# Dunni3/FlowMol

Hardware: AMD Instinct MI355X
Metric: molecules/sec at 250 timesteps (GEOM-drugs-sized graphs) (higher is better)
Workload: dtype f32

## Files before the change

flowmol_amd/csrc/fm_engine.cpp:

```cpp
#include "fm_host.h"

namespace fmh { thread_local std::string g_create_error; }

namespace {

struct Blob {
    const float* base; const fm_tensor_desc* t; int n;
    std::string err;
    const float* get(const std::string& name, int64_t d0, int64_t d1 = -1) {
        for (int i = 0; i < n; ++i)
            if (name == t[i].name) {
                const bool ok = (d1 < 0) ? (t[i].ndim == 1 && t[i].shape[0] == d0)
                                         : (t[i].ndim == 2 && t[i].shape[0] == d0 && t[i].shape[1] == d1);
                if (!ok) {
                    char b[256];
                    snprintf(b, sizeof b, "tensor %s: shape (%lld,%lld) != expected (%lld,%lld)", name.c_str(),
                             (long long)t[i].shape[0], (long long)(t[i].ndim > 1 ? t[i].shape[1] : -1), (long long)d0, (long long)d1);
                    if (err.empty()) err = b;
                    return nullptr;
                }
                return base + t[i].offset;
            }
        if (err.empty()) err = "missing tensor " + name;
        return nullptr;
// ... 184 lines not shown
        else launch_mlp(L, mode_n, node, a, wn, N, p.small_node ? 16 : FM_TM);
        if (pair) launch_mlp(L, mode_p, pair, e, wp, U, p.small_pair ? 16 : pair32 ? 32 : FM_TM);
    }
}

void launch_node_proj(Launch& L, const char* name, int V, bool small, int N, const FmProjArgs& pa) {
    const int tm = small ? 16 : FM_TM;
    launch_inst(L, node_proj_instances, {V, tm}, name, dim3((N + tm - 1) / tm), dim3(FM_THREADS), lds_proj(V, tm), pa);
}

int evaluate(fm_ctx* c, hipStream_t st, const fm_state* state, const fm_dst* prev, int remove_com, const fm_dst* out,
             bool taps_on, const fm_dense_state* dense = nullptr, const float* temb = nullptr) {
    Launch L{c, st};
    const BatchPlan& p = c->plan;
    const int V = c->V, TE = p.tm_edge, TN = p.tm_node, HX = c->HX;
    const FmBatch& b = c->b;
    const int N = b.N, E = b.E, U = b.U;
    const fm_config& cf = c->cfg;
    const int nc1 = c->nc + 1;
    auto tap = [&](const std::string& n, const void* src, size_t bytes) { if (taps_on) L.tap(n, src, bytes); };

    const bool mlp4 = p.mlp4 && !dense;
    const int n_pq = (prev && !dense) ? p.n_pq : 0;
    FmMlpArgs ma{};
    ma.na = c->na; ma.nc = c->nc; ma.ne = c->ne;
    ma.rbf_mu_step = c->rbf_mu_step; ma.rbf_inv_sigma = c->rbf_inv_sigma;
    const float* x_t = dense ? dense->x_t : state->x_t;
    if (dense) {
        const int kp = c->node_embed.K1p;
        L("dense_in", fm_k_dense_node_in, dim3(std::min(2048, (int)(((size_t)N * kp + 255) / 256))), dim3(256), 0, c->Ps, kp, N,
          (const float*)dense->a_t, c->na, (const float*)dense->c_t, c->nc, temb, cf.time_embedding_dim);
        FmMlpArgs a{};
        a.in = c->Ps; a.in_ld = kp; a.out = c->s; a.out_ld = 256; a.ln_g = c->node_ln_g; a.ln_b = c->node_ln_b; a.ln_n = c->S;
        launch_mlp(L, FM_MLP_TABLE, "embed_nodes", a, c->node_embed, N);
        FmMlpArgs e{};
        e.in = dense->e_t; e.in_ld = c->ne; e.in_w = c->ne; e.out = c->ef; e.out_ld = 128; e.ln_g = c->edge_ln_g; e.ln_b = c->edge_ln_b; e.ln_n = c->F;
        e.p_e0 = b.p_e0; e.p_e1 = b.p_e1;
        launch_mlp(L, FM_MLP_TABLE, "embed_pairs", e, c->edge_embed, U);
        tap("embed.s", c->s, (size_t)N * 256 * 4);
        tap("embed.ef", c->ef, (size_t)E * 128 * 4);
    } else if (prev) {
        FmMlpArgs a = ma;
        a.s_tab = c->s_tab; a.tok_a = state->a_t; a.tok_c = state->c_t; a.n_c1 = nc1;
        a.prev_a = prev->a; a.prev_c = prev->c; a.prev_x = prev->x; a.x_t = state->x_t;
        a.out = c->s;
        FmMlpArgs e = ma;
        e.e_src = b.e_src; e.e_dst = b.e_dst; e.e_pair = b.e_pair; e.tok_e = state->e_t;
        e.prev_e = prev->e; e.prev_x = prev->x; e.x_t = state->x_t; e.T1 = c->T1; e.ef_tab = c->ef_tab;
        e.out = c->ef;
        e.p_e0 = b.p_e0; e.p_e1 = b.p_e1;
        if (n_pq > 0) {
            e.slabW0 = c->conv[0].Ws_slab; e.slabQ0 = c->Q[0];
            if (n_pq > 1) { e.slabW1 = c->conv[1].Ws_slab; e.slabQ1 = c->Q[1]; }
        }
        FmMlp4Args a4{};
        a4.N = N; a4.W1q = c->sc_node_W1q; a4.b1 = c->sc_node.b1; a4.W2q = c->sc_node_W2q; a4.b2 = c->sc_node.b2;
        a4.s_tab = a.s_tab; a4.tok_a = a.tok_a; a4.tok_c = a.tok_c; a4.n_c1 = nc1; a4.prev_a = a.prev_a; a4.prev_c = a.prev_c; a4.prev_x = a.prev_x; a4.x_t = a.x_t;
        a4.na = c->na; a4.nc = c->nc; a4.rbf_mu_step = c->rbf_mu_step; a4.rbf_inv_sigma = c->rbf_inv_sigma; a4.out = c->s;
        launch_mlp_stage(L, p, mlp4, FM_MLP4_SC_NODE, FM_MLP_SC_NODE, FM_MLP_SC_EDGE, "sc", "sc_node", "sc_edge", a4, a, c->sc_node, e, c->sc_edge, n_pq > 0);
        tap("sc.s", c->s, (size_t)N * 256 * 4);
        tap("sc.ef", c->ef, (size_t)E * 128 * 4);
    } else {
        L("gather_s", fm_k_gather_rows, dim3(std::min(2048, (N * 64 + 255) / 256)), dim3(256), 0, c->s, (const float*)c->s_tab, 256, N,
          (const int*)state->a_t, (const int*)state->c_t, nc1, (const int*)nullptr);
        L("gather_ef", fm_k_gather_rows, dim3(std::min(4096, (int)(((size_t)E * 32 + 255) / 256))), dim3(256), 0, c->ef, c->ef_tab, 128, E,
          (const int*)state->e_t, (const int*)nullptr, 0, (const int*)b.e_pair);
        tap("embed.s", c->s, (size_t)N * 256 * 4);
        tap("embed.ef", c->ef, (size_t)E * 128 * 4);
    }

    const dim3 blk(FM_THREADS);
    const dim3 gn((N + FM_TM - 1) / FM_TM), ge((E + FM_TM - 1) / FM_TM);
    const dim3 gnt((N + TN - 1) / TN), get(p.n_tiles_msg);
    const bool fuse = p.fuse_node;
    const int n_pass = cf.n_convs * (cf.n_recycles > 1 ? cf.n_recycles : 1);
    bool head_done = false;
    for (int it = 0; it < n_pass; ++it) {
        const int i = it % cf.n_convs;
        const ConvW& cw = c->conv[i];
        if (it == 0 || !fuse) {
            FmProjArgs pa{};
            pa.N = N; pa.s = c->s; pa.v = c->v; pa.Wps = cw.Wps; pa.Ps = c->Ps; pa.Wpv = cw.Wpv; pa.PV = c->PV; pa.pv_w = c->PVW;
            if (it == 0) { pa.v_init = c->v; pa.x_src = x_t; pa.x_dst = c->xw; }
            if (it == 0 && mlp4) {
                FmMlp4Args p4{};
                p4.N = N; p4.in = c->s; p4.Wps4 = cw.Wps4; p4.Ps = c->Ps; p4.PV = c->PV; p4.pv_w = c->PVW; p4.v_init = c->v; p4.V = V; p4.x_src = x_t; p4.x_dst = c->xw;
                launch_inst(L, mlp4_instances, {FM_MLP4_PROJ0}, "node_proj", dim3((N + 3) / 4), blk, (size_t)FM_MLP4_LDS_BYTES, p4);
            }
            else launch_node_proj(L, "node_proj", V, p.small_node, N, pa);
        }
        FmMsgArgs m{};
        m.b = b; m.x = c->xw; m.ef = c->ef; m.Ps = c->Ps; m.PV = c->PV; m.w0 = cw.w0;
        if (HX > 0) {
            FmDstProjArgs dp{};
            dp.N = N; dp.s = c->s; dp.v = c->v; dp.g = cw.dproj; dp.Wsd = cw.Wsd; dp.Psd = c->Psd; dp.Wpvd = cw.Wpvd; dp.PVd = c->PVd; dp.pv_w = c->PVW;
            fm_launch_dst_proj(L, V, TN, HX, gnt, dp);
            m.Psd = c->Psd; m.PVd = c->PVd;
        }
        m.g0 = cw.msg[0]; m.g1 = cw.msg[1]; m.g2 = cw.msg[2];
        m.part_s = c->part_s; m.part_v = c->part_v;
        m.rbf_mu_step = c->rbf_mu_step; m.rbf_inv_sigma = c->rbf_inv_sigma;
        const bool dbg = taps_on && it == 0 && c->taps.count("conv0.msg.s") && c->taps.count("conv0.msg.v");
        m.dbg_s = dbg ? (float*)c->taps["conv0.msg.s"] : nullptr; m.dbg_v = dbg ? (float*)c->taps["conv0.msg.v"] : nullptr;
        dim3 gmsg = get;
        if (p.xcd_swizzle) { m.xcd_chunk = ((int)get.x + 7) / 8; gmsg = dim3(8 * m.xcd_chunk); }
        const bool pq = it < n_pq;
        if (pq) { m.Q = c->Q[it]; m.g0.Ws = cw.Ws_sh; }
        fm_launch_edge_message(L, V, TE, HX, cf.precision, pq, gmsg, m);
        const int u = cf.update_after[i];
        FmNodeUpdArgs nu{};
        nu.b = b; nu.s = c->s; nu.v = c->v; nu.part_s = c->part_s; nu.part_v = c->part_v; nu.inv_z = cf.msg_z < 0.f ? -1.0f : 1.0f / cf.msg_z;
        nu.g0 = cw.upd[0]; nu.g1 = cw.upd[1]; nu.g2 = cw.upd[2];
        nu.ln1_g = cw.ln1_g; nu.ln1_b = cw.ln1_b; nu.ln2_g = cw.ln2_g; nu.ln2_b = cw.ln2_b;
        const std::string ci = "conv" + std::to_string(i);
        const bool tagg = taps_on && (c->taps.count(ci + ".agg.s") || c->taps.count(ci + ".agg.v"));
// ... 13 lines not shown
                if (u >= 0) nu.Wasd_sp = c->upd[u].Wasd_sp;
            }
            const int rg = p.node_rg;
            const size_t lds = p.node_sp ? lds_gvp_sp(V, TN) - (size_t)TN * 9 * 4 : lds_gvp(V, TN, false);
            fm_launch_node_update(L, V, TN, p.node_sp || c->mp.narrow_s, p.node_sp, rg, rg ? dim3((N + 4 * rg - 1) / (4 * rg)) : gnt, lds, nu);
        }
        if (tagg) { tap(ci + ".agg.s", c->tap_s, (size_t)N * 256 * 4); tap(ci + ".agg.v", c->tap_v, (size_t)N * 3 * V * 4); }
        tap(ci + ".s", c->s, (size_t)N * 256 * 4);
        tap(ci + ".v", c->v, (size_t)N * 3 * V * 4);
        if (u >= 0) {
            const UpdW& uw = c->upd[u];
            if (!fuse) {
                FmPosArgs pp{};
                pp.N = N; pp.s = c->s; pp.v = c->v; pp.x = c->xw; pp.g0 = uw.pos[0]; pp.g1 = uw.pos[1]; pp.g2 = uw.pos[2];
                fm_launch_pos_update(L, V, TN, gnt, pp);
                FmProjArgs pa2{};
                pa2.N = N; pa2.s = c->s; pa2.v = c->v; pa2.Wasd = uw.Wasd; pa2.Asd = c->Asd;
                launch_node_proj(L, "node_proj_asd", V, p.small_node, N, pa2);
            }
            FmEdgeUpdArgs eu{};
            eu.b = b; eu.x = c->xw; eu.Asd = c->Asd; eu.ef = c->ef; eu.W1 = uw.W1; eu.b1 = uw.b1; eu.W2 = uw.W2; eu.b2 = uw.b2;
            eu.ln_g = uw.ln_g; eu.ln_b = uw.ln_b; eu.rbf_mu_step = c->rbf_mu_step; eu.rbf_inv_sigma = c->rbf_inv_sigma;
            eu.f_real = c->F;
            if (c->mp.node_sp) {
                const FmEdgeUpdSpW sw{uw.W1_sp, uw.W2_sp};
                launch_inst(L, edge_update_sp_instances, {32, c->mp.half_planes}, "edge_update", dim3((E + 31) / 32), blk, lds_edge_upd_sp(32), eu, sw);
            } else if (it == n_pass - 1 && p.fuse_head && !(taps_on && c->taps.count("upd" + std::to_string(i) + ".ef"))) {
                eu.hW1 = c->edge_head.W1; eu.hb1 = c->edge_head.b1; eu.hW2 = c->edge_head.W2; eu.hb2 = c->edge_head.b2; eu.out_e = out->e; eu.ne = c->ne;
                launch_inst(L, edge_update_instances, {32, false, true}, "edge_update_head", dim3((U + 15) / 16), blk, lds_edge_upd(32), eu);
                head_done = true;
            } else {
                const int tm = p.tm_eupd;
                launch_inst(L, edge_update_instances, {tm, c->mp.narrow_f, false}, "edge_update", dim3((E + tm - 1) / tm), blk, lds_edge_upd(tm), eu);
            }
            const std::string ui = "upd" + std::to_string(i);
            tap(ui + ".x", c->xw, (size_t)N * 3 * 4);
            if (!head_done) tap(ui + ".ef", c->ef, (size_t)E * 128 * 4);
        }
    }
    {
        FmMlpArgs a = ma;
        a.in = c->s; a.out = out->a; a.out2 = out->c;
        FmMlpArgs e = ma;
        e.ef = c->ef; e.p_e0 = b.p_e0; e.p_e1 = b.p_e1; e.out = out->e;
        FmMlp4Args a4{};
        a4.N = N; a4.W1q = c->node_head_W1q; a4.b1 = c->node_head.b1; a4.W2q = c->node_head_W2q; a4.b2 = c->node_head.b2;
        a4.na = c->na; a4.nc = c->nc; a4.in = c->s; a4.out = out->a; a4.out2 = out->c;
        launch_mlp_stage(L, p, mlp4, FM_MLP4_NODE_HEAD, FM_MLP_NODE_HEAD, FM_MLP_EDGE_HEAD, "heads", "node_head", head_done ? nullptr : "edge_head", a4, a, c->node_head,
                         e, c->edge_head, p.edge_head32);
    }
    if (remove_com != 2) {
        L.copy(out->x, c->xw, (size_t)N * 3 * 4);
        if (remove_com) L("remove_com", fm_k_remove_com, dim3(b.B), dim3(64), 0, out->x, (const int*)b.mol_node_off);
    }
    return L.rc;
// ... 415 lines not shown
    if (tn == 4 || tn == 8 || tn == 12 || tn == 20) {
        if (m.quad_node) p.node_rg = tn / 4;
        tn = tn == 20 ? 32 : 16;
    }
    p.tm_node = tn;
    if ((c->HX || !cf.has_mask) && (p.tm_node > 32)) p.tm_node = 32;
    p.node_sp = p.fuse_node && p.tm_node <= 32 ? m.node_sp : 0;
    p.tm_eupd = cf.tile_edge_update == 64 && !m.narrow_f && !m.node_sp ? 64 : 32;
    p.fuse_head = (cf.fuse_node == 0 || cf.fuse_node == 1) && !m.narrow_f && p.tm_eupd == 32 && !m.node_sp
                  && (long long)nmax * (nmax - 1) * 512 < 0x7ffffe00LL;
    if (U > 0 && (cf.pair_slab > 0 || cf.canonical >= 0 || (U + 31) / 32 >= 16LL * n_cus)) p.n_pq = m.slab_convs;
    const int mlp_tiles = (p.N + FM_TM - 1) / FM_TM + (U + FM_TM - 1) / FM_TM;
    p.pair_mlps = cf.fuse_node >= 0 && (cf.pair_mlps ? cf.pair_mlps > 0 : mlp_tiles <= n_cus);
    p.small_node = cf.mlp_small_tiles ? cf.mlp_small_tiles > 0 : (p.N + 15) / 16 <= 4 * n_cus;
    p.small_pair = cf.mlp_small_tiles ? cf.mlp_small_tiles > 0 : (U + 15) / 16 <= 4 * n_cus;
    p.mlp4 = m.quad_mlp && (cf.mlp_small_tiles ? cf.mlp_small_tiles == 2 : (p.N + 3) / 4 <= n_cus);
    p.edge_head32 = (U + 31) / 32 >= 16 * n_cus;
    p.ctmc_threads = (B * 4 <= n_cus && nmax > 23) || nmax >= 92 ? 1024 : 256;
    return FM_OK;
}

struct WsLayout {
    size_t off_mol_tile, off_tile_desc, off_mol_node, off_mol_edge, off_mol_pair, off_node_mol, off_first_edge, off_esrc, off_edst, off_epair, off_pe0, off_pe1,
        off_pair_mol, off_s, off_v, off_xw, off_ef, off_Ps, off_Asd, off_PV, off_part_s, off_part_v, off_Psd, off_PVd, off_stab, off_bx, off_ba,
        off_bc, off_be, off_tap_s, off_tap_v, off_gid, off_sa1, off_sc1, off_se1, off_Q0, off_Q1, total;
};

static WsLayout ws_layout(const fm_ctx* c, const BatchPlan& p) {
    const size_t B = p.B, N = p.N, E = p.E, U = p.U, V = c->V;
    WsLayout w;
    size_t o = 0;
    auto take = [&](size_t bytes) { size_t r = o; o = align_up(o + bytes, 256); return r; };
    w.off_mol_tile = take((B + 1) * 4); w.off_tile_desc = take((size_t)p.n_tiles_msg * 16);
    w.off_mol_node = take((B + 1) * 4); w.off_mol_edge = take((B + 1) * 4); w.off_mol_pair = take((B + 1) * 4);
    w.off_node_mol = take(N * 4); w.off_first_edge = take(N * 4);
    w.off_esrc = take(E * 4); w.off_edst = take(E * 4); w.off_epair = take(E * 4);
    w.off_pe0 = take(U * 4); w.off_pe1 = take(U * 4); w.off_pair_mol = take(U * 4);
    w.off_s = take(N * 256 * 4); w.off_v = take(N * 3 * V * 4); w.off_xw = take(N * 3 * 4);
    w.off_ef = take(E * 128 * 4);
    w.off_Ps = take(N * 256 * 4); w.off_Asd = take(N * 256 * 4); w.off_PV = take(N * 3 * c->PVW * 4);
    w.off_Psd = take(c->HX ? N * 256 * 4 : 0); w.off_PVd = take(c->HX ? N * 3 * c->PVW * 4 : 0);
    w.off_part_s = take(N * p.P * 256 * 4); w.off_part_v = take(N * p.P * 3 * V * 4);
    w.off_stab = take(align_up(c->tab_rows, FM_TM) * 256 * 4 * FM_TAB_SLOTS);
    w.off_bx = take(N * 3 * 4); w.off_ba = take(N * c->na * 4); w.off_bc = take(N * c->nc * 4); w.off_be = take(U * c->ne * 4);
    w.off_tap_s = take(N * 256 * 4); w.off_tap_v = take(N * 3 * V * 4);
    w.off_gid = take(B * 4);
    w.off_sa1 = take(N * 4); w.off_sc1 = take(N * 4); w.off_se1 = take(U * 4);
    w.off_Q0 = take(p.n_pq > 0 ? U * 256 * 4 : 0); w.off_Q1 = take(p.n_pq > 1 ? U * 256 * 4 : 0);
    w.total = o;
    return w;
}

int fm_workspace_bytes(fm_ctx* c, const int32_t* n_atoms, int B, size_t* bytes) {
    if (!c || !n_atoms || !bytes) return fail(c, FM_ERR_INVALID, "fm_workspace_bytes: null argument");
    BatchPlan p;
    const int rc = plan_batch(c, n_atoms, B, p);
    if (rc) return rc;
    *bytes = ws_layout(c, p).total;
    return FM_OK;
}
// ... 38 lines not shown
    for (int i = 0; i < B; ++i) {
        const int n = n_atoms[i];
        no[i + 1] = no[i] + n; eo[i + 1] = eo[i] + n * (n - 1); po[i + 1] = po[i] + n * (n - 1) / 2; ids[i] = i;
        to[i + 1] = to[i] + (n * (n - 1) + p.tm_edge - 1) / p.tm_edge;
    }
    {
        hipError_t e_ = hipMemcpyAsync(base + w.off_mol_node, no, (size_t)(B + 1) * 4, hipMemcpyHostToDevice, st);
        if (e_ == hipSuccess) e_ = hipMemcpyAsync(base + w.off_mol_edge, eo, (size_t)(B + 1) * 4, hipMemcpyHostToDevice, st);
        if (e_ == hipSuccess) e_ = hipMemcpyAsync(base + w.off_mol_pair, po, (size_t)(B + 1) * 4, hipMemcpyHostToDevice, st);
        if (e_ == hipSuccess) e_ = hipMemcpyAsync(base + w.off_mol_tile, to, (size_t)(B + 1) * 4, hipMemcpyHostToDevice, st);
        if (e_ == hipSuccess) e_ = hipMemcpyAsync(base + w.off_gid, ids, (size_t)B * 4, hipMemcpyHostToDevice, st);
        rc = stage_release(c, st);
        if (e_ != hipSuccess) return fail(c, FM_ERR_HIP, "fm_batch_bind: descriptor copy failed: %s", hipGetErrorString(e_));
        if (rc) return rc;
    }
    FmBatch& b = c->b;
    b.B = B; b.N = p.N; b.E = p.E; b.U = p.U; b.P = p.P;
    b.n_tiles = p.n_tiles_msg; b.tile_rows = p.tm_edge;
    b.mol_tile_off = (const int*)(base + w.off_mol_tile); b.tile_desc = (int4*)(base + w.off_tile_desc);
    b.mol_node_off = (const int*)(base + w.off_mol_node); b.mol_edge_off = (const int*)(base + w.off_mol_edge); b.mol_pair_off = (const int*)(base + w.off_mol_pair);
    b.node_mol = (int*)(base + w.off_node_mol); b.node_first_edge = (int*)(base + w.off_first_edge);
    b.e_src = (int*)(base + w.off_esrc); b.e_dst = (int*)(base + w.off_edst); b.e_pair = (int*)(base + w.off_epair);
    b.p_e0 = (int*)(base + w.off_pe0); b.p_e1 = (int*)(base + w.off_pe1); b.pair_mol = (int*)(base + w.off_pair_mol);
    c->s = (float*)(base + w.off_s); c->v = (float*)(base + w.off_v); c->xw = (float*)(base + w.off_xw); c->ef = (float*)(base + w.off_ef);
    c->Ps = (float*)(base + w.off_Ps); c->Asd = (float*)(base + w.off_Asd); c->PV = (float*)(base + w.off_PV);
    c->part_s = (float*)(base + w.off_part_s); c->part_v = (float*)(base + w.off_part_v);
    c->Psd = (float*)(base + w.off_Psd); c->PVd = (float*)(base + w.off_PVd);
    c->s_tab = c->s_tab_base = (float*)(base + w.off_stab);
    c->tab_slot_floats = (size_t)align_up(c->tab_rows, FM_TM) * 256;
    c->boot.x = (float*)(base + w.off_bx); c->boot.a = (float*)(base + w.off_ba); c->boot.c = (float*)(base + w.off_bc); c->boot.e = (float*)(base + w.off_be);
    c->tap_s = (float*)(base + w.off_tap_s); c->tap_v = (float*)(base + w.off_tap_v);
    c->mol_gid = (int*)(base + w.off_gid);
    c->sa1 = (int32_t*)(base + w.off_sa1); c->sc1 = (int32_t*)(base + w.off_sc1); c->se1 = (int32_t*)(base + w.off_se1);
    c->Q[0] = (float*)(base + w.off_Q0); c->Q[1] = (float*)(base + w.off_Q1);
    Launch L{c, st};
    const int work = p.E > p.N ? p.E : p.N;
    L("batch_setup", fm_k_batch_setup, dim3((work + 255) / 256), dim3(256), 0, b);
    if (L.rc) return L.rc;
    c->bound = true; c->plan = p;
    return FM_OK;
}

int fm_remove_com(fm_ctx* c, void* stream, float* x) {
    if (!c || !x) return fail(c, FM_ERR_INVALID, "fm_remove_com: null argument");
    if (!c->bound) return fail(c, FM_ERR_STATE, "fm_remove_com: no batch bound");
    Launch L{c, (hipStream_t)stream};
// ... 109 lines not shown
        cur ^= 1;
    }
    if (final_dst) *final_dst = cur ^ 1;
    return FM_OK;
}

int fm_set_tap(fm_ctx* c, const char* name, void* dst) {
    if (!c || !name) return fail(c, FM_ERR_INVALID, "fm_set_tap: null argument");
    if (dst) c->taps[name] = dst; else c->taps.erase(name);
    return FM_OK;
}
int fm_clear_taps(fm_ctx* c) { if (c) c->taps.clear(); return FM_OK; }

int fm_batch_query(fm_ctx* c, void* stream, const char* name, int32_t* dst) {
    if (!c || !name || !dst) return fail(c, FM_ERR_INVALID, "fm_batch_query: null argument");
    if (!c->bound) return fail(c, FM_ERR_STATE, "fm_batch_query: no batch bound");
    const FmBatch& b = c->b;
    const std::string n = name;
    const int* src = nullptr; size_t cnt = 0;
    if (n == "e_src") { src = b.e_src; cnt = b.E; } else if (n == "e_dst") { src = b.e_dst; cnt = b.E; }
    else if (n == "e_pair") { src = b.e_pair; cnt = b.E; } else if (n == "p_e0") { src = b.p_e0; cnt = b.U; }
    else if (n == "p_e1") { src = b.p_e1; cnt = b.U; } else if (n == "node_mol") { src = b.node_mol; cnt = b.N; }
    else if (n == "pair_mol") { src = b.pair_mol; cnt = b.U; }
    else return fail(c, FM_ERR_INVALID, "fm_batch_query: unknown array %s", name);
    FM_HIP(c, hipMemcpyAsync(dst, src, cnt * 4, hipMemcpyDeviceToDevice, (hipStream_t)stream));
    return FM_OK;
}

#ifdef FM_TRACE
int fm_trace_read(unsigned long long* out) { (void)hipMemcpyFromSymbol(out, HIP_SYMBOL(fm_trace), 16384 * 16 * 8); return 0; }
#endif
#ifdef FM_PHASE_TIMING
int fm_tlog_read(unsigned long long* out, int reset) {
    (void)hipMemcpyFromSymbol(out, HIP_SYMBOL(fm_tlog), 64 * 8);
    if (reset) { unsigned long long z[64] = {0}; (void)hipMemcpyToSymbol(HIP_SYMBOL(fm_tlog), z, 64 * 8); }
    return 0;
}
#endif

int fm_stability(fm_ctx* c, void* stream, const fm_state* state, const uint32_t* table, int n_types, int fake_atom_token,
                 int explicit_aromaticity, int32_t* out) {
    if (!c || !state || !table || !out) return fail(c, FM_ERR_INVALID, "fm_stability: null argument");
    if (!c->bound) return fail(c, FM_ERR_STATE, "fm_stability: no batch bound");
    if (!state->a_t || !state->c_t || !state->e_t) return fail(c, FM_ERR_INVALID, "fm_stability: state tokens missing");
    Launch L{c, (hipStream_t)stream};
    FmStabArgs a{};
// ... 35 lines not shown
```

flowmol_amd/csrc/fm_host.h:

```cpp
#pragma once
#include <hip/hip_runtime.h>

#include <algorithm>
#include <array>
#include <cmath>
#include <cstdarg>
#include <cstdint>
#include <cstdio>
#include <cstdlib>
#include <cstring>
#include <functional>
#include <map>
#include <memory>
#include <string>
#include <vector>

#include "../../include/flowmol_hip.h"
#include "fm_kernels.h"

namespace fmh {

constexpr int FM_TAB_SLOTS = 32;

extern thread_local std::string g_create_error;
// ... 55 lines not shown
using namespace fmh;

struct fm_ctx {
    fm_config cfg{};
    std::string err;
    int V = 32, S = 256, F = 128, na = 0, nc = 0, ne = 0;
    int HX = 0, SD = 0, PVW = 48;
    int n_cus = 256;
    ModelPlan mp{};
    const void *sc_node_W1q = nullptr, *sc_node_W2q = nullptr, *node_head_W1q = nullptr, *node_head_W2q = nullptr;
    float* Q[2] = {nullptr, nullptr};
    float rbf_mu_step = 0.f, rbf_inv_sigma = 0.f;
    char* arena = nullptr; size_t arena_bytes = 0;
    const float *emb_a = nullptr, *emb_c = nullptr;
    MlpW node_embed{}, edge_embed{}, sc_node{}, sc_edge{}, node_head{}, edge_head{};
    const float *node_ln_g = nullptr, *node_ln_b = nullptr, *edge_ln_g = nullptr, *edge_ln_b = nullptr;
    const float *ef_tab = nullptr, *T1 = nullptr;
    std::vector<ConvW> conv;
    std::vector<UpdW> upd;
    int tab_rows = 0;
    bool bound = false;
    BatchPlan plan{};
    FmBatch b{};
    float *s = nullptr, *v = nullptr, *xw = nullptr, *ef = nullptr, *Ps = nullptr, *Asd = nullptr, *PV = nullptr;
    float *part_s = nullptr, *part_v = nullptr, *s_tab = nullptr, *Psd = nullptr, *PVd = nullptr;
    float* s_tab_base = nullptr; size_t tab_slot_floats = 0;
    float *tap_s = nullptr, *tap_v = nullptr;
    fm_dst boot{};
    int32_t *sa1 = nullptr, *sc1 = nullptr, *se1 = nullptr;
    int* mol_gid = nullptr;
    int32_t* stage = nullptr; size_t stage_cap = 0; hipEvent_t stage_ev = nullptr; bool stage_busy = false;
    std::map<std::string, void*> taps;
    bool prof = false;
    std::vector<hipEvent_t> ev_pool;
    std::vector<ProfEvent> prof_events;
    std::vector<std::string> prof_names;
    std::map<std::string, std::pair<double, int64_t>> prof_acc;
};

namespace fmh {

inline int fail(fm_ctx* c, int code, const char* fmt, ...) {
    char buf[1024];
    va_list ap; va_start(ap, fmt); vsnprintf(buf, sizeof buf, fmt, ap); va_end(ap);
    if (c) c->err = buf; else g_create_error = buf;
    return code;
// ... 98 lines not shown
```

flowmol_amd/csrc/fm_kernels.h:

```cpp
#pragma once
#include <type_traits>

#include "fm_device.h"

struct FmBatch {
    int B, N, E, U;
    int P;
    int n_tiles, tile_rows;
    const int* mol_node_off;
    const int* mol_edge_off;
    const int* mol_pair_off;
    int* node_mol;
    int* node_first_edge;
    int* e_src;
    int* e_dst;
    int* e_pair;
    int* p_e0;
    int* p_e1;
    int* pair_mol;
    const int* mol_tile_off;
    int4* tile_desc;
};

#define FM_CHUNK_E 16

static __global__ void __launch_bounds__(256) fm_k_batch_setup(FmBatch b) {
    const int gid = blockIdx.x * blockDim.x + threadIdx.x;
    if (gid < b.N) {
        int lo = 0, hi = b.B;
        while (hi - lo > 1) { const int mid = (lo + hi) >> 1; if (b.mol_node_off[mid] <= gid) lo = mid; else hi = mid; }
        b.node_mol[gid] = lo;
        const int n = b.mol_node_off[lo + 1] - b.mol_node_off[lo];
        b.node_first_edge[gid] = b.mol_edge_off[lo] + (gid - b.mol_node_off[lo]) * (n - 1);
    }
    if (gid < b.E) {
        int lo = 0, hi = b.B;
        while (hi - lo > 1) { const int mid = (lo + hi) >> 1; if (b.mol_edge_off[mid] <= gid) lo = mid; else hi = mid; }
        const int noff = b.mol_node_off[lo];
        const int n = b.mol_node_off[lo + 1] - noff;
        const int local = gid - b.mol_edge_off[lo];
        const int i = local / (n - 1), k = local % (n - 1);
        const int j = k + (k >= i ? 1 : 0);
        b.e_dst[gid] = noff + i;
        b.e_src[gid] = noff + j;
        const int a = i < j ? i : j, c = i < j ? j : i;
        const int pair = b.mol_pair_off[lo] + a * (2 * n - a - 1) / 2 + (c - a - 1);
        b.e_pair[gid] = pair;
        if (j < i) { b.p_e0[pair] = gid; b.pair_mol[pair] = lo; }
        else b.p_e1[pair] = gid;
    }
    if (gid < b.n_tiles) {
        int lo = 0, hi = b.B;
        while (hi - lo > 1) { const int mid = (lo + hi) >> 1; if (b.mol_tile_off[mid] <= gid) lo = mid; else hi = mid; }
        const int moff = b.mol_edge_off[lo];
        const int e0 = moff + (gid - b.mol_tile_off[lo]) * b.tile_rows;
        const int left = b.mol_edge_off[lo + 1] - e0;
        b.tile_desc[gid] = make_int4(e0, left < b.tile_rows ? left : b.tile_rows, moff, lo);
    }
}

enum FmMlpMode {
    FM_MLP_TABLE = 0,
    FM_MLP_SC_NODE = 1,
    FM_MLP_NODE_HEAD = 2,
    FM_MLP_EDGE_HEAD = 3,
    FM_MLP_SC_EDGE = 4,
};

struct FmMlpArgs {
    int rows;
    int K1p;
    int H;
    int O;
    int ldx, ldh;
    const float2* W1; const float* b1;
    const float2* W2; const float* b2;
    const float* ln_g; const float* ln_b; int ln_n;
    const float* in;  int in_ld;
    int in_w;
    float* out; int out_ld;
    const float* s_tab; const int* tok_a; const int* tok_c; int n_c1;
    const float* prev_a; const float* prev_c; const float* prev_x; const float* x_t;
    int na, nc, ne;
    float rbf_mu_step, rbf_inv_sigma;
    float* out2;
    const float* ef; const int* p_e0; const int* p_e1;
    const int* e_src; const int* e_dst; const int* e_pair; const int* tok_e;
    const float* prev_e; const float* T1; const float* ef_tab;
    const float* emb_a; const float* emb_c; const float* temb; int ta, tc, tt;
    const float2* slabW0; float* slabQ0; const float2* slabW1; float* slabQ1;
    int tab_tiles; int tab_stride;
};

template <int MODE, int TM>
__device__ __forceinline__ void fm_mlp2_tile(const FmMlpArgs& a, int tile, float* lds) {
    float* X = lds;
    float* Hb = lds + TM * a.ldx;
    int* meta = reinterpret_cast<int*>(Hb + TM * a.ldh);
    const int tid = threadIdx.x;
    const int row0 = tile * TM;

    if (MODE == FM_MLP_TABLE) {
        for (int idx = tid; idx < TM * a.K1p; idx += FM_THREADS) {
            const int r = idx / a.K1p, c = idx % a.K1p, row = row0 + r;
            float v = 0.f;
            if (row < a.rows) {
                if (a.in) v = (a.in_w == 0 || c < a.in_w) ? a.in[(size_t)row * a.in_ld + c] : 0.f;
                else {
                    const int ia = row / a.n_c1, ic = row % a.n_c1;
                    if (c < a.ta) v = a.emb_a ? a.emb_a[ia * a.ta + c] : (c == ia ? 1.f : 0.f);
                    else if (c < a.ta + a.tc) v = a.emb_c ? a.emb_c[ic * a.tc + (c - a.ta)] : ((c - a.ta) == ic ? 1.f : 0.f);
                    else if (c < a.ta + a.tc + a.tt) v = a.temb[c - a.ta - a.tc];
                }
// ... 69 lines not shown
            u0[k] = reinterpret_cast<const float4*>(a.ef)[(size_t)(ea < 0 ? 0 : ea) * 32 + c4];
            u1[k] = reinterpret_cast<const float4*>(a.ef)[(size_t)(eb < 0 ? 0 : eb) * 32 + c4];
        }
#pragma unroll
        for (int k = 0; k < NQ; ++k) {
            const int idx = tid + k * FM_THREADS, r = idx >> 5, c4 = idx & 31;
            const bool ok = meta[r] >= 0;
            float4 v;
            v.x = ok ? u0[k].x + u1[k].x : 0.f; v.y = ok ? u0[k].y + u1[k].y : 0.f;
            v.z = ok ? u0[k].z + u1[k].z : 0.f; v.w = ok ? u0[k].w + u1[k].w : 0.f;
            *reinterpret_cast<float4*>(X + r * a.ldx + 4 * c4) = v;
        }
    } else {
        float* dd = reinterpret_cast<float*>(meta + TM);
        int* pr = meta + 3 * TM;
        if (tid < TM) {
            const int p = row0 + tid;
            int tok = -1, ea = -1, eb = -1;
            float dt_ = 0.f, d1_ = 0.f;
            if (p < a.rows) {
                ea = a.p_e0[p]; eb = a.p_e1[p];
                const int i = a.e_src[ea], j = a.e_dst[ea];
                tok = a.tok_e[p];
                dt_ = fm_norm3(a.x_t[i * 3] - a.x_t[j * 3], a.x_t[i * 3 + 1] - a.x_t[j * 3 + 1], a.x_t[i * 3 + 2] - a.x_t[j * 3 + 2]) + 1e-8f;
                d1_ = fm_norm3(a.prev_x[i * 3] - a.prev_x[j * 3], a.prev_x[i * 3 + 1] - a.prev_x[j * 3 + 1],
                               a.prev_x[i * 3 + 2] - a.prev_x[j * 3 + 2]) + 1e-8f;
            }
            meta[tid] = tok; pr[tid] = eb; dd[2 * tid] = dt_; dd[2 * tid + 1] = d1_;
            meta[4 * TM + tid] = ea;
        }
        __syncthreads();
        for (int idx = tid; idx < TM * a.K1p; idx += FM_THREADS) {
            const int r = idx / a.K1p, c = idx % a.K1p;
            float v = 0.f;
            if (meta[r] >= 0) {
                if (c < a.ne) v = a.prev_e[(size_t)(row0 + r) * a.ne + c];
                else if (c < a.ne + 32)
                    v = fm_rbf(dd[2 * r + 1], c - a.ne, a.rbf_mu_step, a.rbf_inv_sigma) -
                        fm_rbf(dd[2 * r], c - a.ne, a.rbf_mu_step, a.rbf_inv_sigma);
            }
            X[r * a.ldx + c] = v;
        }
    }
    __syncthreads();

    fm_block_gemm<TM / 16, 1>(X, a.ldx, TM / 16, a.K1p / 8, a.W1, a.H / 16, [&](int row, int col, float v) {
        if (MODE == FM_MLP_SC_EDGE) { const int t = meta[row]; v += (t >= 0) ? a.T1[t * 128 + col] : 0.f; }
// ... 342 lines not shown
        if (row0 + row < a.N) a.Psd[(size_t)(row0 + row) * 256 + col] = val;
    });
    fm_block_gemm<1, 1>(Vin, T::LDVI, 3 * MT, 1, a.Wpvd, a.pv_w / 16, [&](int row, int col, float val) {
        const int c = row / TM, r = row % TM;
        if (row0 + r < a.N) a.PVd[((size_t)(row0 + r) * 3 + c) * a.pv_w + col] = val;
    });
}

struct FmMsgArgs {
    FmBatch b;
    const float* x;
    const float* ef;
    const float* Ps;
    const float* PV;
    const float* w0;
    const float* Psd;
    const float* PVd;
    FmGvpW g0, g1, g2;
    float* part_s;
    float* part_v;
    float rbf_mu_step, rbf_inv_sigma;
    float* dbg_s; float* dbg_v;
    const float* Q;
    int xcd_chunk;
};

template <int V, int TM, int NTH, int HX, int SP, int PQ = 0>
__global__ void __launch_bounds__(NTH) fm_k_edge_message(FmMsgArgs a) {
    static_assert(!(PQ && (SP || HX)), "the pair-slab instance exists for f32 models without destination features");
    typedef FmGvpTile<V, TM, HX> T;
    HIP_DYNAMIC_SHARED(float, lds)
    float* X = lds;
    constexpr int FMT = SP == 3 ? 1 : 0, NPL = SP == 2 ? 3 : 2;
    float* Vin = X + (SP ? TM * FM_LDP * NPL / 2 : T::X_FLOATS);
    float* Vh = Vin + T::VIN_FLOATS;
    float* G = SP ? Vh + TM * FM_LDG : Vh + T::VH_FLOATS;
    int* m_src = reinterpret_cast<int*>(SP ? Vh + T::VH_FLOATS : G + T::G_FLOATS);
    int* m_dst = m_src + TM;
    float* m_geo = reinterpret_cast<float*>(m_dst + TM);
    int* m_piece = reinterpret_cast<int*>(m_geo + 4 * TM);
    int* m_soff = m_piece + TM;
    int* m_doff = m_soff + TM;
    const int tid = threadIdx.x;
    const int tile = a.xcd_chunk > 0 ? (int)(blockIdx.x & 7) * a.xcd_chunk + (int)(blockIdx.x >> 3) : (int)blockIdx.x;
    if (tile >= a.b.n_tiles) return;
    const int4 td = a.b.tile_desc[tile];
    const int e0 = td.x, left = td.y, moff = td.z;
    FM_MARK_DECL
    constexpr int NEF = PQ ? 1 : TM * 32 / NTH;
    float4 efv[NEF];
    if constexpr (!PQ) {
        const auto rs = fm_buf(a.ef + (size_t)e0 * 128, (unsigned)left * 512u);
#pragma unroll
        for (int k = 0; k < NEF; ++k) efv[k] = (FM_ABLATE & 16) ? make_float4(0.1f, 0.2f, 0.3f, 0.4f) : fm_buf_f32x4(rs, tid * 16 + k * NTH * 16, 0);
    }
    if (PQ && tid < 64) {
        const int e = e0 + tid;
        const int pr = tid < left ? a.b.e_pair[e] : 0x7fffffff;
        int mn = pr;
#pragma unroll
        for (int o = 1; o < 64; o <<= 1) { const int t = __shfl_xor(mn, o); mn = t < mn ? t : mn; }
        if (tid < TM) m_doff[tid] = pr != 0x7fffffff ? (pr - mn) * 1024 : FM_BUF_OOB;
        if (tid == 0) m_doff[TM] = mn;
    }
    if (tid < TM) {
        const int e = e0 + tid;
        int s = -1, d = -1, piece = 0;
        float gx = 0.f, gy = 0.f, gz = 0.f, dist = 0.f;
        if (tid < left) {
            s = a.b.e_src[e]; d = a.b.e_dst[e];
            piece = (e - moff) / FM_CHUNK_E - (a.b.node_first_edge[d] - moff) / FM_CHUNK_E;
            const float dx = a.x[s * 3] - a.x[d * 3], dy = a.x[s * 3 + 1] - a.x[d * 3 + 1], dz = a.x[s * 3 + 2] - a.x[d * 3 + 2];
            dist = fm_norm3(dx, dy, dz) + 1e-8f;
            const float inv_d = __builtin_amdgcn_rcpf(dist);
            gx = dx * inv_d; gy = dy * inv_d; gz = dz * inv_d;
        }
        m_src[tid] = s; m_dst[tid] = d; m_piece[tid] = piece;
        m_soff[tid] = s >= 0 ? s * 1024 : FM_BUF_OOB;
        if (!PQ) m_doff[tid] = d >= 0 ? d * 1024 : FM_BUF_OOB;
        m_geo[4 * tid] = gx; m_geo[4 * tid + 1] = gy; m_geo[4 * tid + 2] = gz; m_geo[4 * tid + 3] = dist;
    }
    __syncthreads();
    FM_MARK(0);
    float pre[TM / 16][1024 / NTH][4];
    if (!(FM_ABLATE & 16)) fm_gather_pre<TM, NTH, false>(pre, a.Ps, a.b.N, m_soff);
    else { for (auto& p1 : pre) for (auto& p2 : p1) for (auto& p3 : p2) p3 = 0.25f; }
    if (HX > 0) fm_gather_pre<TM, NTH, true>(pre, a.Psd, a.b.N, m_doff);
    float preq[PQ ? TM / 16 : 1][PQ ? 1024 / NTH : 1][4];
    if constexpr (PQ) {
        static_assert(!PQ || NTH == 512, "Q rows are laid out for 8 waves x 2 column tiles");
        const int pmin = __builtin_amdgcn_readfirstlane(m_doff[TM]);
        const int lane = tid & 63, wave = __builtin_amdgcn_readfirstlane(tid >> 6);
        const auto rs = fm_buf(a.Q + (size_t)pmin * 256, 0x7ffffc00u);
#pragma unroll
        for (int i = 0; i < TM / 16; ++i)
#pragma unroll
            for (int r = 0; r < 4; ++r) {
                const float2 t = fm_buf_f32x2(rs, m_doff[i * 16 + 4 * (lane >> 4) + r] + (lane & 15) * 8, wave * 128);
                preq[i][0][r] = t.x; preq[i][1][r] = t.y;
            }
    }
    {
        constexpr int PVW = T::PVW, CB = PVW / 16, NCH = 3 * CB * TM, QN = NTH / 16, NP = (NCH + QN - 1) / QN;
// ... 396 lines not shown
            if (idx < NCHK) {
                const int r = idx / (3 * V4), rem = idx % (3 * V4), c = rem / V4, u4 = rem % V4;
                *reinterpret_cast<float4*>(Vin + (c * TM + r) * T::LDVI + u4 * 4) = qv[k];
            }
        }
    }
    __syncthreads();
    {
        FM_MARK_DECL
        float pre[TM / 16][2][4];
        fm_gvp_core<V, V, false, true, TM, FM_THREADS>(X, Vin, Vh, G, a.g0, pre FM_MARK_PASS(50));
        fm_gvp_core<V, V, false, true, TM, FM_THREADS>(X, Vin, Vh, G, a.g1, pre FM_MARK_PASS(50));
        fm_gvp_core<V, 1, false, false, TM, FM_THREADS>(X, Vin, Vh, G, a.g2, pre FM_MARK_PASS(50));
    }
    if (tid < TM * 3) {
        const int r = tid / 3, c = tid % 3, n = row0 + r;
        if (n < a.N) a.x[n * 3 + c] += Vin[(c * TM + r) * T::LDVI];
    }
}

struct FmEdgeUpdArgs {
    FmBatch b;
    const float* x;
    const float* Asd;
    float* ef;
    const float2* W1; const float* b1;
    const float2* W2; const float* b2;
    const float* ln_g; const float* ln_b;
    float rbf_mu_step, rbf_inv_sigma;
    int f_real;
    const float2* hW1; const float* hb1;
    const float2* hW2; const float* hb2;
    float* out_e; int ne;
};

template <int TM, bool NARROW, bool HEAD = false>
__global__ void __launch_bounds__(FM_THREADS) fm_k_edge_update(FmEdgeUpdArgs a) {
    static_assert(!HEAD || (TM == 32 && !NARROW), "the fused edge head exists for 32-row tiles of full-width models");
    HIP_DYNAMIC_SHARED(float, lds)
    constexpr int LDX = 164, LDH = 132, MT = TM / 16, LPR = FM_THREADS / TM;
    float* X = lds;
    float* Hb = lds + TM * LDX;
    int* m_soff = reinterpret_cast<int*>(Hb + TM * LDH);
    int* m_doff = m_soff + TM;
    float* m_d = reinterpret_cast<float*>(m_doff + TM);
    const int tid = threadIdx.x, lane = tid & 63, wave = __builtin_amdgcn_readfirstlane(tid >> 6), e0 = blockIdx.x * TM;
    constexpr int NEF = TM * 32 / FM_THREADS;
    float4 efv[NEF];
    const int left = a.b.E - e0;
    const auto rs_ef = fm_buf(a.ef + (size_t)(HEAD ? 0 : e0) * 128, HEAD ? 0u : (unsigned)(left < TM ? left : TM) * 512u);
    if constexpr (!HEAD) {
#pragma unroll
        for (int k = 0; k < NEF; ++k) efv[k] = fm_buf_f32x4(rs_ef, tid * 16 + k * FM_THREADS * 16, 0);
    }
    int* m_eoff = reinterpret_cast<int*>(m_d + TM);
    if (HEAD && tid < 64) {
        const int p = blockIdx.x * (TM / 2) + (tid >> 1);
        const int e = (tid < TM && p < a.b.U) ? ((tid & 1) ? a.b.p_e1[p] : a.b.p_e0[p]) : 0x7fffffff;
        int mn = e;
#pragma unroll
        for (int o = 1; o < 64; o <<= 1) { const int t = __shfl_xor(mn, o); mn = t < mn ? t : mn; }
        if (tid < TM) {
            int s = -1, d = -1; float dist = 0.f;
            if (e != 0x7fffffff) {
                s = a.b.e_src[e]; d = a.b.e_dst[e];
                dist = fm_norm3(a.x[s * 3] - a.x[d * 3], a.x[s * 3 + 1] - a.x[d * 3 + 1], a.x[s * 3 + 2] - a.x[d * 3 + 2]) + 1e-8f;
            }
            m_soff[tid] = s >= 0 ? s * 1024 : FM_BUF_OOB; m_doff[tid] = s >= 0 ? d * 1024 : FM_BUF_OOB; m_d[tid] = dist;
            m_eoff[tid] = s >= 0 ? (e - mn) * 512 : FM_BUF_OOB;
        }
        if (tid == 0) m_eoff[TM] = mn;
    }
    if (!HEAD && tid < TM) {
        const int e = e0 + tid;
        int s = -1, d = -1; float dist = 0.f;
        if (e < a.b.E) {
            s = a.b.e_src[e]; d = a.b.e_dst[e];
            dist = fm_norm3(a.x[s * 3] - a.x[d * 3], a.x[s * 3 + 1] - a.x[d * 3 + 1], a.x[s * 3 + 2] - a.x[d * 3 + 2]) + 1e-8f;
        }
        m_soff[tid] = s >= 0 ? s * 1024 : FM_BUF_OOB; m_doff[tid] = s >= 0 ? d * 1024 : FM_BUF_OOB; m_d[tid] = dist;
    }
    __syncthreads();
    if constexpr (HEAD) {
        const int emin = __builtin_amdgcn_readfirstlane(m_eoff[TM]);
        const auto rs_g = fm_buf(a.ef + (size_t)(emin == 0x7fffffff ? 0 : emin) * 128, 0x7ffffe00u);
#pragma unroll
        for (int k = 0; k < NEF; ++k) {
            const int idx = tid + k * FM_THREADS;
            efv[k] = fm_buf_f32x4(rs_g, m_eoff[idx >> 5] + (idx & 31) * 16, 0);
        }
    }
    const int col = wave * 16 + (lane & 15);
    float pre_s[MT][4], pre_d[MT][4];
    const float b1 = a.b1[col], b2 = a.b2[col];
    {
        const auto rs = fm_buf(a.Asd, (unsigned)a.b.N * 1024u);
#pragma unroll
        for (int i = 0; i < MT; ++i) {
            const int4 so = *reinterpret_cast<const int4*>(m_soff + i * 16 + 4 * (lane >> 4)), dof = *reinterpret_cast<const int4*>(m_doff + i * 16 + 4 * (lane >> 4));
            const int so_[4] = {so.x, so.y, so.z, so.w}, do_[4] = {dof.x, dof.y, dof.z, dof.w};
#pragma unroll
// ... 515 lines not shown
```

flowmol_amd/engine.py:

```python
from __future__ import annotations

import ctypes as C
import math
from dataclasses import dataclass
from typing import Callable, Dict, List, Optional, Sequence

import torch

from . import _lib
from ._lib import (FM_DFM_CAMPBELL, FM_DFM_GAT, FM_NOISE_PHILOX, FlowMolHipError, fm_dense_state, fm_endpoint_scalars, fm_config, fm_dst, fm_sampled, fm_state, fm_step_noise, fm_step_scalars,
                   fm_tensor_desc, fm_traj_sink)
from .config import VFConfig
from .weights import check_state_dict, state_dict_shapes


def _ptr(t: Optional[torch.Tensor]):
    return None if t is None else C.c_void_p(t.data_ptr())


def time_embedding_host(t: float, dim: int) -> torch.Tensor:
    tt = torch.tensor([t], dtype=torch.float32)
    if dim == 1:
        return tt.clone()
    ts = tt * 1000
# ... 251 lines not shown
        if n.dim() != 1 or n.numel() == 0:
            raise ValueError('n_atoms must be a non-empty 1-D tensor')
        need = C.c_size_t()
        self._check(self.lib.fm_workspace_bytes(self._ctx, C.c_void_p(n.data_ptr()), n.numel(), C.byref(need)), 'fm_workspace_bytes')
        if self._ws is None or self._ws.numel() < need.value:
            self._ws = None
            self._ws = torch.empty(need.value + 256, dtype=torch.uint8, device=self.device)
        base = self._ws.data_ptr()
        aligned = (base + 255) // 256 * 256
        with self._dev():
            self._check(self.lib.fm_batch_bind(self._ctx, self._stream(), C.c_void_p(n.data_ptr()), n.numel(),
                                               C.c_void_p(aligned), need.value), 'fm_batch_bind')
        n64 = n.to(torch.int64)
        self.n_atoms = n64
        self.B = int(n.numel())
        self.N = int(n64.sum())
        self.E = int((n64 * (n64 - 1)).sum())
        self.U = self.E // 2
        self.workspace_bytes = int(need.value)
        return self

    def query(self, name: str) -> torch.Tensor:
        cnt = {'e_src': self.E, 'e_dst': self.E, 'e_pair': self.E, 'p_e0': self.U, 'p_e1': self.U,
               'node_mol': self.N, 'pair_mol': self.U}[name]
        out = torch.empty(cnt, dtype=torch.int32, device=self.device)
        with self._dev():
            self._check(self.lib.fm_batch_query(self._ctx, self._stream(), name.encode(), _ptr(out)), 'fm_batch_query')
        self.synchronize()
        return out

    def new_dst(self) -> Dict[str, torch.Tensor]:
        d = self.device
        return {'x': torch.empty(self.N, 3, device=d), 'a': torch.empty(self.N, self.cfg.n_atom_types, device=d),
                'c': torch.empty(self.N, self.cfg.n_charges, device=d), 'e': torch.empty(self.U, self.cfg.n_bond_types, device=d)}

    @staticmethod
    def _dst_struct(d) -> fm_dst:
        s = fm_dst()
        s.x, s.a, s.c, s.e = _ptr(d['x']), _ptr(d['a']), _ptr(d['c']), _ptr(d['e'])
        return s

    @staticmethod
    def _state_struct(st) -> fm_state:
        s = fm_state()
        s.x_t, s.a_t, s.c_t, s.e_t = _ptr(st['x_t']), _ptr(st['a_t']), _ptr(st['c_t']), _ptr(st['e_t'])
        return s

# ... 221 lines not shown
```

Measured before the change: 62.97.

## Precompute per-edge metadata and cache edge geometry across edge kernels

Adds a packed int4 per-edge metadata array (src, dst, piece, pair) built once at batch bind, and a float4 per-edge geometry buffer (unit vector plus distance). The self-conditioning edge MLP and the edge update kernel write this buffer, and the message kernel reads it instead of gathering coordinates and recomputing norms. This replaces several scattered index loads and recomputation with one vectorized load per edge. In exchange it adds workspace memory and extra global writes, and it relies on a validity flag that tracks when positions change.

Result: no change. 63.11 (median of 6 runs) (+0.2%).

```diff
diff --git a/flowmol_amd/csrc/fm_engine.cpp b/flowmol_amd/csrc/fm_engine.cpp
--- a/flowmol_amd/csrc/fm_engine.cpp
+++ b/flowmol_amd/csrc/fm_engine.cpp
@@ -230,6 +230,8 @@
 
     const bool mlp4 = p.mlp4 && !dense;
     const int n_pq = (prev && !dense) ? p.n_pq : 0;
+    const bool geo_tab = cf.precision == FM_PREC_F32;
+    bool geo_ok = false;
     FmMlpArgs ma{};
     ma.na = c->na; ma.nc = c->nc; ma.ne = c->ne;
     ma.rbf_mu_step = c->rbf_mu_step; ma.rbf_inv_sigma = c->rbf_inv_sigma;
@@ -257,6 +259,7 @@
         e.prev_e = prev->e; e.prev_x = prev->x; e.x_t = state->x_t; e.T1 = c->T1; e.ef_tab = c->ef_tab;
         e.out = c->ef;
         e.p_e0 = b.p_e0; e.p_e1 = b.p_e1;
+        if (geo_tab) { e.geo = c->geo; geo_ok = true; }
         if (n_pq > 0) {
             e.slabW0 = c->conv[0].Ws_slab; e.slabQ0 = c->Q[0];
             if (n_pq > 1) { e.slabW1 = c->conv[1].Ws_slab; e.slabQ1 = c->Q[1]; }
@@ -298,7 +301,7 @@
             else launch_node_proj(L, "node_proj", V, p.small_node, N, pa);
         }
         FmMsgArgs m{};
-        m.b = b; m.x = c->xw; m.ef = c->ef; m.Ps = c->Ps; m.PV = c->PV; m.w0 = cw.w0;
+        m.b = b; m.x = c->xw; m.geo = geo_ok ? c->geo : nullptr; m.ef = c->ef; m.Ps = c->Ps; m.PV = c->PV; m.w0 = cw.w0;
         if (HX > 0) {
             FmDstProjArgs dp{};
             dp.N = N; dp.s = c->s; dp.v = c->v; dp.g = cw.dproj; dp.Wsd = cw.Wsd; dp.Psd = c->Psd; dp.Wpvd = cw.Wpvd; dp.PVd = c->PVd; dp.pv_w = c->PVW;
@@ -358,6 +361,7 @@
             eu.b = b; eu.x = c->xw; eu.Asd = c->Asd; eu.ef = c->ef; eu.W1 = uw.W1; eu.b1 = uw.b1; eu.W2 = uw.W2; eu.b2 = uw.b2;
             eu.ln_g = uw.ln_g; eu.ln_b = uw.ln_b; eu.rbf_mu_step = c->rbf_mu_step; eu.rbf_inv_sigma = c->rbf_inv_sigma;
             eu.f_real = c->F;
+            geo_ok = false;
             if (c->mp.node_sp) {
                 const FmEdgeUpdSpW sw{uw.W1_sp, uw.W2_sp};
                 launch_inst(L, edge_update_sp_instances, {32, c->mp.half_planes}, "edge_update", dim3((E + 31) / 32), blk, lds_edge_upd_sp(32), eu, sw);
@@ -367,6 +371,7 @@
                 head_done = true;
             } else {
                 const int tm = p.tm_eupd;
+                if (geo_tab) { eu.geo = c->geo; geo_ok = true; }
                 launch_inst(L, edge_update_instances, {tm, c->mp.narrow_f, false}, "edge_update", dim3((E + tm - 1) / tm), blk, lds_edge_upd(tm), eu);
             }
             const std::string ui = "upd" + std::to_string(i);
@@ -828,7 +833,7 @@
 
 struct WsLayout {
     size_t off_mol_tile, off_tile_desc, off_mol_node, off_mol_edge, off_mol_pair, off_node_mol, off_first_edge, off_esrc, off_edst, off_epair, off_pe0, off_pe1,
-        off_pair_mol, off_s, off_v, off_xw, off_ef, off_Ps, off_Asd, off_PV, off_part_s, off_part_v, off_Psd, off_PVd, off_stab, off_bx, off_ba,
+        off_pair_mol, off_emeta, off_geo, off_s, off_v, off_xw, off_ef, off_Ps, off_Asd, off_PV, off_part_s, off_part_v, off_Psd, off_PVd, off_stab, off_bx, off_ba,
         off_bc, off_be, off_tap_s, off_tap_v, off_gid, off_sa1, off_sc1, off_se1, off_Q0, off_Q1, total;
 };
 
@@ -842,6 +847,7 @@
     w.off_node_mol = take(N * 4); w.off_first_edge = take(N * 4);
     w.off_esrc = take(E * 4); w.off_edst = take(E * 4); w.off_epair = take(E * 4);
     w.off_pe0 = take(U * 4); w.off_pe1 = take(U * 4); w.off_pair_mol = take(U * 4);
+    w.off_emeta = take(E * 16); w.off_geo = take(E * 16);
     w.off_s = take(N * 256 * 4); w.off_v = take(N * 3 * V * 4); w.off_xw = take(N * 3 * 4);
     w.off_ef = take(E * 128 * 4);
     w.off_Ps = take(N * 256 * 4); w.off_Asd = take(N * 256 * 4); w.off_PV = take(N * 3 * c->PVW * 4);
@@ -926,6 +932,7 @@
     b.node_mol = (int*)(base + w.off_node_mol); b.node_first_edge = (int*)(base + w.off_first_edge);
     b.e_src = (int*)(base + w.off_esrc); b.e_dst = (int*)(base + w.off_edst); b.e_pair = (int*)(base + w.off_epair);
     b.p_e0 = (int*)(base + w.off_pe0); b.p_e1 = (int*)(base + w.off_pe1); b.pair_mol = (int*)(base + w.off_pair_mol);
+    b.e_meta = (int4*)(base + w.off_emeta); c->geo = (float4*)(base + w.off_geo);
     c->s = (float*)(base + w.off_s); c->v = (float*)(base + w.off_v); c->xw = (float*)(base + w.off_xw); c->ef = (float*)(base + w.off_ef);
     c->Ps = (float*)(base + w.off_Ps); c->Asd = (float*)(base + w.off_Asd); c->PV = (float*)(base + w.off_PV);
     c->part_s = (float*)(base + w.off_part_s); c->part_v = (float*)(base + w.off_part_v);
@@ -1081,6 +1088,8 @@
     else if (n == "e_pair") { src = b.e_pair; cnt = b.E; } else if (n == "p_e0") { src = b.p_e0; cnt = b.U; }
     else if (n == "p_e1") { src = b.p_e1; cnt = b.U; } else if (n == "node_mol") { src = b.node_mol; cnt = b.N; }
     else if (n == "pair_mol") { src = b.pair_mol; cnt = b.U; }
+    else if (n == "e_meta") { src = (const int*)b.e_meta; cnt = (size_t)b.E * 4; }
+    else if (n == "e_geo") { src = (const int*)c->geo; cnt = (size_t)b.E * 4; }
     else return fail(c, FM_ERR_INVALID, "fm_batch_query: unknown array %s", name);
     FM_HIP(c, hipMemcpyAsync(dst, src, cnt * 4, hipMemcpyDeviceToDevice, (hipStream_t)stream));
     return FM_OK;
diff --git a/flowmol_amd/csrc/fm_host.h b/flowmol_amd/csrc/fm_host.h
--- a/flowmol_amd/csrc/fm_host.h
+++ b/flowmol_amd/csrc/fm_host.h
@@ -101,6 +101,7 @@
     bool bound = false;
     BatchPlan plan{};
     FmBatch b{};
+    float4* geo = nullptr;
     float *s = nullptr, *v = nullptr, *xw = nullptr, *ef = nullptr, *Ps = nullptr, *Asd = nullptr, *PV = nullptr;
     float *part_s = nullptr, *part_v = nullptr, *s_tab = nullptr, *Psd = nullptr, *PVd = nullptr;
     float* s_tab_base = nullptr; size_t tab_slot_floats = 0;
diff --git a/flowmol_amd/csrc/fm_kernels.h b/flowmol_amd/csrc/fm_kernels.h
--- a/flowmol_amd/csrc/fm_kernels.h
+++ b/flowmol_amd/csrc/fm_kernels.h
@@ -20,6 +20,7 @@
     int* pair_mol;
     const int* mol_tile_off;
     int4* tile_desc;
+    int4* e_meta;
 };
 
 #define FM_CHUNK_E 16
@@ -46,6 +47,7 @@
         const int a = i < j ? i : j, c = i < j ? j : i;
         const int pair = b.mol_pair_off[lo] + a * (2 * n - a - 1) / 2 + (c - a - 1);
         b.e_pair[gid] = pair;
+        b.e_meta[gid] = make_int4(noff + j, noff + i, local / FM_CHUNK_E - (i * (n - 1)) / FM_CHUNK_E, pair);
         if (j < i) { b.p_e0[pair] = gid; b.pair_mol[pair] = lo; }
         else b.p_e1[pair] = gid;
     }
@@ -89,6 +91,7 @@
     const float* prev_e; const float* T1; const float* ef_tab;
     const float* emb_a; const float* emb_c; const float* temb; int ta, tc, tt;
     const float2* slabW0; float* slabQ0; const float2* slabW1; float* slabQ1;
+    float4* geo;
     int tab_tiles; int tab_stride;
 };
 
@@ -204,7 +207,13 @@
                 ea = a.p_e0[p]; eb = a.p_e1[p];
                 const int i = a.e_src[ea], j = a.e_dst[ea];
                 tok = a.tok_e[p];
-                dt_ = fm_norm3(a.x_t[i * 3] - a.x_t[j * 3], a.x_t[i * 3 + 1] - a.x_t[j * 3 + 1], a.x_t[i * 3 + 2] - a.x_t[j * 3 + 2]) + 1e-8f;
+                const float dx = a.x_t[i * 3] - a.x_t[j * 3], dy = a.x_t[i * 3 + 1] - a.x_t[j * 3 + 1], dz = a.x_t[i * 3 + 2] - a.x_t[j * 3 + 2];
+                dt_ = fm_norm3(dx, dy, dz) + 1e-8f;
+                if (a.geo) {
+                    const float inv_d = __builtin_amdgcn_rcpf(dt_);
+                    a.geo[ea] = make_float4(dx * inv_d, dy * inv_d, dz * inv_d, dt_);
+                    a.geo[eb] = make_float4((a.x_t[j * 3] - a.x_t[i * 3]) * inv_d, (a.x_t[j * 3 + 1] - a.x_t[i * 3 + 1]) * inv_d, (a.x_t[j * 3 + 2] - a.x_t[i * 3 + 2]) * inv_d, dt_);
+                }
                 d1_ = fm_norm3(a.prev_x[i * 3] - a.prev_x[j * 3], a.prev_x[i * 3 + 1] - a.prev_x[j * 3 + 1],
                                a.prev_x[i * 3 + 2] - a.prev_x[j * 3 + 2]) + 1e-8f;
             }
@@ -593,6 +602,7 @@
     float rbf_mu_step, rbf_inv_sigma;
     float* dbg_s; float* dbg_v;
     const float* Q;
+    const float4* geo;
     int xcd_chunk;
 };
 
@@ -616,7 +626,7 @@
     const int tile = a.xcd_chunk > 0 ? (int)(blockIdx.x & 7) * a.xcd_chunk + (int)(blockIdx.x >> 3) : (int)blockIdx.x;
     if (tile >= a.b.n_tiles) return;
     const int4 td = a.b.tile_desc[tile];
-    const int e0 = td.x, left = td.y, moff = td.z;
+    const int e0 = td.x, left = td.y;
     FM_MARK_DECL
     constexpr int NEF = PQ ? 1 : TM * 32 / NTH;
     float4 efv[NEF];
@@ -625,31 +635,34 @@
 #pragma unroll
         for (int k = 0; k < NEF; ++k) efv[k] = (FM_ABLATE & 16) ? make_float4(0.1f, 0.2f, 0.3f, 0.4f) : fm_buf_f32x4(rs, tid * 16 + k * NTH * 16, 0);
     }
-    if (PQ && tid < 64) {
-        const int e = e0 + tid;
-        const int pr = tid < left ? a.b.e_pair[e] : 0x7fffffff;
-        int mn = pr;
-#pragma unroll
-        for (int o = 1; o < 64; o <<= 1) { const int t = __shfl_xor(mn, o); mn = t < mn ? t : mn; }
-        if (tid < TM) m_doff[tid] = pr != 0x7fffffff ? (pr - mn) * 1024 : FM_BUF_OOB;
-        if (tid == 0) m_doff[TM] = mn;
-    }
-    if (tid < TM) {
-        const int e = e0 + tid;
-        int s = -1, d = -1, piece = 0;
-        float gx = 0.f, gy = 0.f, gz = 0.f, dist = 0.f;
-        if (tid < left) {
-            s = a.b.e_src[e]; d = a.b.e_dst[e];
-            piece = (e - moff) / FM_CHUNK_E - (a.b.node_first_edge[d] - moff) / FM_CHUNK_E;
-            const float dx = a.x[s * 3] - a.x[d * 3], dy = a.x[s * 3 + 1] - a.x[d * 3 + 1], dz = a.x[s * 3 + 2] - a.x[d * 3 + 2];
-            dist = fm_norm3(dx, dy, dz) + 1e-8f;
-            const float inv_d = __builtin_amdgcn_rcpf(dist);
-            gx = dx * inv_d; gy = dy * inv_d; gz = dz * inv_d;
-        }
-        m_src[tid] = s; m_dst[tid] = d; m_piece[tid] = piece;
-        m_soff[tid] = s >= 0 ? s * 1024 : FM_BUF_OOB;
-        if (!PQ) m_doff[tid] = d >= 0 ? d * 1024 : FM_BUF_OOB;
-        m_geo[4 * tid] = gx; m_geo[4 * tid + 1] = gy; m_geo[4 * tid + 2] = gz; m_geo[4 * tid + 3] = dist;
+    if (tid < 64) {
+        int s = -1, d = -1, piece = 0, pr = 0x7fffffff;
+        float4 g = make_float4(0.f, 0.f, 0.f, 0.f);
+        if (tid < TM && tid < left) {
+            const int e = e0 + tid;
+            const int4 mt = a.b.e_meta[e];
+            s = mt.x; d = mt.y; piece = mt.z; pr = mt.w;
+            if (a.geo) g = a.geo[e];
+            else {
+                const float dx = a.x[s * 3] - a.x[d * 3], dy = a.x[s * 3 + 1] - a.x[d * 3 + 1], dz = a.x[s * 3 + 2] - a.x[d * 3 + 2];
+                g.w = fm_norm3(dx, dy, dz) + 1e-8f;
+                const float inv_d = __builtin_amdgcn_rcpf(g.w);
+                g.x = dx * inv_d; g.y = dy * inv_d; g.z = dz * inv_d;
+            }
+        }
+        if constexpr (PQ != 0) {
+            int mn = pr;
+#pragma unroll
+            for (int o = 1; o < 64; o <<= 1) { const int t = __shfl_xor(mn, o); mn = t < mn ? t : mn; }
+            if (tid < TM) m_doff[tid] = pr != 0x7fffffff ? (pr - mn) * 1024 : FM_BUF_OOB;
+            if (tid == 0) m_doff[TM] = mn;
+        }
+        if (tid < TM) {
+            m_src[tid] = s; m_dst[tid] = d; m_piece[tid] = piece;
+            m_soff[tid] = s >= 0 ? s * 1024 : FM_BUF_OOB;
+            if (!PQ) m_doff[tid] = d >= 0 ? d * 1024 : FM_BUF_OOB;
+            m_geo[4 * tid] = g.x; m_geo[4 * tid + 1] = g.y; m_geo[4 * tid + 2] = g.z; m_geo[4 * tid + 3] = g.w;
+        }
     }
     __syncthreads();
     FM_MARK(0);
@@ -1092,6 +1105,7 @@
 struct FmEdgeUpdArgs {
     FmBatch b;
     const float* x;
+    float4* geo;
     const float* Asd;
     float* ef;
     const float2* W1; const float* b1;
@@ -1133,7 +1147,8 @@
         if (tid < TM) {
             int s = -1, d = -1; float dist = 0.f;
             if (e != 0x7fffffff) {
-                s = a.b.e_src[e]; d = a.b.e_dst[e];
+                const int4 mt = a.b.e_meta[e];
+                s = mt.x; d = mt.y;
                 dist = fm_norm3(a.x[s * 3] - a.x[d * 3], a.x[s * 3 + 1] - a.x[d * 3 + 1], a.x[s * 3 + 2] - a.x[d * 3 + 2]) + 1e-8f;
             }
             m_soff[tid] = s >= 0 ? s * 1024 : FM_BUF_OOB; m_doff[tid] = s >= 0 ? d * 1024 : FM_BUF_OOB; m_d[tid] = dist;
@@ -1145,8 +1160,14 @@
         const int e = e0 + tid;
         int s = -1, d = -1; float dist = 0.f;
         if (e < a.b.E) {
-            s = a.b.e_src[e]; d = a.b.e_dst[e];
-            dist = fm_norm3(a.x[s * 3] - a.x[d * 3], a.x[s * 3 + 1] - a.x[d * 3 + 1], a.x[s * 3 + 2] - a.x[d * 3 + 2]) + 1e-8f;
+            const int4 mt = a.b.e_meta[e];
+            s = mt.x; d = mt.y;
+            const float dx = a.x[s * 3] - a.x[d * 3], dy = a.x[s * 3 + 1] - a.x[d * 3 + 1], dz = a.x[s * 3 + 2] - a.x[d * 3 + 2];
+            dist = fm_norm3(dx, dy, dz) + 1e-8f;
+            if (a.geo) {
+                const float inv_d = __builtin_amdgcn_rcpf(dist);
+                a.geo[e] = make_float4(dx * inv_d, dy * inv_d, dz * inv_d, dist);
+            }
         }
         m_soff[tid] = s >= 0 ? s * 1024 : FM_BUF_OOB; m_doff[tid] = s >= 0 ? d * 1024 : FM_BUF_OOB; m_d[tid] = dist;
     }
diff --git a/flowmol_amd/engine.py b/flowmol_amd/engine.py
--- a/flowmol_amd/engine.py
+++ b/flowmol_amd/engine.py
@@ -297,7 +297,7 @@
 
     def query(self, name: str) -> torch.Tensor:
         cnt = {'e_src': self.E, 'e_dst': self.E, 'e_pair': self.E, 'p_e0': self.U, 'p_e1': self.U,
-               'node_mol': self.N, 'pair_mol': self.U}[name]
+               'node_mol': self.N, 'pair_mol': self.U, 'e_meta': 4 * self.E, 'e_geo': 4 * self.E}[name]
         out = torch.empty(cnt, dtype=torch.int32, device=self.device)
         with self._dev():
             self._check(self.lib.fm_batch_query(self._ctx, self._stream(), name.encode(), _ptr(out)), 'fm_batch_query')
```
